# TencentARC/HOSNeRF

Measured on AMD Instinct MI355X. Metric: train rays/sec (stage3: forward + losses + backward + gradient all-reduce + Adam; LPIPS term OFF in this line -- stages.stage3_with_lpips carries it), higher is better.
Workload: dtype f32 (fp16/bf16 hi-lo split MFMA x3, fp32 accumulate)

## Files before the change

### hosnerf_amd/csrc/hos_mlpbwd.hip

```cpp
#include "hos_gemm_common.h"
#include <cstdlib>
#include <type_traits>
#include <utility>

namespace {

typedef __bf16 bf16x8 __attribute__((ext_vector_type(8)));
typedef __bf16 bf16x4 __attribute__((ext_vector_type(4)));
typedef short s16x4 __attribute__((ext_vector_type(4)));
typedef short s16x8 __attribute__((ext_vector_type(8)));

struct MlpBwdArgs {
    const float* dZ; int lddz;
    const float* X; int ldx;
    const float* W; int ldw;
    float* dX; int lddx;
    float* dW; int lddw;
    float* db;
    int M, N, K;
    int relu_mask;
    float* ws;
    int ws_dw;
    const int* m_dev;
};
// ... 272 lines not shown
                for (int q = 0; q < 4; ++q)
                    if (t * 4 + q < a.N) __hip_atomic_fetch_add(a.db + t * 4 + q, sv[q], __ATOMIC_RELAXED, __HIP_MEMORY_SCOPE_AGENT);
            }
        }
    }
#ifdef HOS_MB_TRACE
    asm volatile("s_waitcnt vmcnt(0)" ::: "memory");
    MB_STAMP();
#endif
#undef MB_STAMP
}

template <int KT>
__global__ __launch_bounds__(MB_NT, 1) void wgrad_tr_fast_kernel(MlpBwdArgs a) {
    constexpr int NT = 8, N_ = NT * 32, K_ = KT * 32, R = 32;
    constexpr int PZ = N_ * 2 + 32, PX = K_ * 2 + 32;
    constexpr int Z_PLANE = R * PZ, X_PLANE = R * PX;
    constexpr int ZU = R * (N_ / 4) / MB_NT;
    constexpr int XT = R * (K_ / 4);
    constexpr int XU = (XT + MB_NT - 1) / MB_NT;
    constexpr bool XALL = XT % MB_NT == 0;
    constexpr int WT = NT * KT, WPW = WT / 8;
    static_assert(WT % 8 == 0 && 8 % KT == 0, "a wave's WGRAD tiles share kt");

    extern __shared__ __attribute__((aligned(16))) char smem_mb[];
    char* const Zh = smem_mb;
    char* const Zl = Zh + Z_PLANE;
    char* const Xh = Zl + Z_PLANE;
    char* const Xl = Xh + X_PLANE;
    const int t = threadIdx.x, lane = t & 63, wave = t >> 6;
    const int tr_g = lane >> 4, tr_p = lane & 15;
    const int tr_row = 8 * (tr_g >> 1) + (tr_p >> 2);
    const int tr_col = 16 * (tr_g & 1) + 4 * (tr_p & 3);
    const bool xthread = XALL || t < XT;

    const int nrb = a.M / R;
    const int G = gridDim.x;
    float4 rzA[ZU], rxA[XU], rzB[ZU], rxB[XU];
    float4 bsum = make_float4(0.f, 0.f, 0.f, 0.f);
    auto gload = [&](float4 (&rz)[ZU], float4 (&rx)[XU], int rb) {
        rb = rb < nrb ? rb : nrb - 1;
        const float* zb = a.dZ + (size_t)rb * R * a.lddz;
        const float* xb = a.X + (size_t)rb * R * a.ldx;
#pragma unroll
        for (int i = 0; i < ZU; ++i) {
            const int u = t + MB_NT * i, row = u / (N_ / 4), c4 = u % (N_ / 4);
            rz[i] = ldg4(zb + (size_t)row * a.lddz + c4 * 4);
        }
#pragma unroll
        for (int i = 0; i < XU; ++i) {
            const int u = XALL ? t + MB_NT * i : (t < XT ? t : 0), row = u / (K_ / 4), c4 = u % (K_ / 4);
            rx[i] = ldg4(xb + (size_t)row * a.ldx + c4 * 4);
        }
    };
    auto sstore = [&](const float4 (&rz)[ZU], const float4 (&rx)[XU]) {
#pragma unroll
        for (int i = 0; i < ZU; ++i) {
            const int u = t + MB_NT * i, row = u / (N_ / 4), c4 = u % (N_ / 4);
            bsum.x += rz[i].x; bsum.y += rz[i].y; bsum.z += rz[i].z; bsum.w += rz[i].w;
            bf16x4 h, l;
            split4(rz[i], h, l);
            *reinterpret_cast<bf16x4*>(Zh + row * PZ + c4 * 8) = h;
            *reinterpret_cast<bf16x4*>(Zl + row * PZ + c4 * 8) = l;
        }
        if (xthread) {
#pragma unroll
            for (int i = 0; i < XU; ++i) {
                const int u = t + MB_NT * i, row = u / (K_ / 4), c4 = u % (K_ / 4);
                bf16x4 h, l;
                split4(rx[i], h, l);
                *reinterpret_cast<bf16x4*>(Xh + row * PX + c4 * 8) = h;
                *reinterpret_cast<bf16x4*>(Xl + row * PX + c4 * 8) = l;
            }
        }
    };
    f32x16 accW[WPW];
#pragma unroll
    for (int j = 0; j < WPW; ++j)
#pragma unroll
        for (int r = 0; r < 16; ++r) accW[j][r] = 0.f;
    auto compute = [&]() {
        const int kw = wave % KT;
        const char* xfrag = Xh + tr_row * PX + (kw * 32 + tr_col) * 2;
#pragma unroll
        for (int s = 0; s < R / 16; ++s) {
            const bf16x8 bh = tr_frag2(xfrag + s * 16 * PX, PX);
            const bf16x8 bl = tr_frag2(xfrag + X_PLANE + s * 16 * PX, PX);
#pragma unroll
            for (int j = 0; j < WPW; ++j) {
                const int ti = wave + 8 * j;
                const char* zfrag = Zh + tr_row * PZ + ((ti / KT) * 32 + tr_col) * 2;
                const bf16x8 ah = tr_frag2(zfrag + s * 16 * PZ, PZ);
                const bf16x8 al = tr_frag2(zfrag + Z_PLANE + s * 16 * PZ, PZ);
                accW[j] = mma3(ah, al, bh, bl, accW[j]);
            }
        }
    };
#define WG_BAR() asm volatile("s_waitcnt lgkmcnt(0)\n\ts_barrier" ::: "memory")
    auto step = [&](float4 (&rz)[ZU], float4 (&rx)[XU], const int rb) {
        sstore(rz, rx);
        WG_BAR();
        gload(rz, rx, rb + 2 * G);
        compute();
        WG_BAR();
    };
    int rb = blockIdx.x;
    gload(rzA, rxA, rb);
    gload(rzB, rxB, rb + G);
    step(rzA, rxA, rb);
    rb += G;
    if (rb < nrb) {
        step(rzB, rxB, rb);
        rb += G;
        while (rb + G < nrb) {
            step(rzA, rxA, rb);
            step(rzB, rxB, rb + G);
            rb += 2 * G;
        }
        if (rb < nrb) step(rzA, rxA, rb);
    }
#undef WG_BAR
    GemmArgs ew{};
    ew.C = a.ws + (size_t)blockIdx.x * (N_ * K_ + N_); ew.ldc = K_; ew.M = N_; ew.N = K_; ew.epi = HOS_EPI_NONE;
#pragma unroll
    for (int j = 0; j < WPW; ++j) {
        const int ti = wave + 8 * j;
        gemm_epilogue_tile<MODE_FWD>(ew, accW[j], (ti / KT) * 32, (ti % KT) * 32, lane);
    }
    if (a.db != nullptr) {
        float4* red = reinterpret_cast<float4*>(Zh);
        red[t] = bsum;
        __syncthreads();
        constexpr int CG = N_ / 4;
        if (t < CG) {
            float4 sacc = make_float4(0.f, 0.f, 0.f, 0.f);
            for (int k = t; k < MB_NT; k += CG) { const float4 v = red[k]; sacc.x += v.x; sacc.y += v.y; sacc.z += v.z; sacc.w += v.w; }
            *reinterpret_cast<float4*>(a.ws + (size_t)blockIdx.x * (N_ * K_ + N_) + N_ * K_ + t * 4) = sacc;
        }
    }
}

constexpr int MB_RSPLIT = 2;
__global__ __launch_bounds__(256) void mlp_bwd_reduce_kernel(const float* __restrict__ ws, int slabs, int n_, int k_, int nk, float* __restrict__ dW,
                                                             int lddw, float* __restrict__ db, int N, int K) {
    const int e = (blockIdx.x * 256 + threadIdx.x) * 4;
    const int slab = nk + n_;
    if (e >= slab || (e >= nk && db == nullptr)) return;
    float4 s = make_float4(0.f, 0.f, 0.f, 0.f);
    const int sy = gridDim.y;
    for (int g0 = blockIdx.y; g0 < slabs; g0 += 8 * sy) {
        float4 v[8];
#pragma unroll
        for (int i = 0; i < 8; ++i) {
            const int g = g0 + i * sy;
            v[i] = g < slabs ? *reinterpret_cast<const float4*>(ws + (size_t)g * slab + e) : make_float4(0.f, 0.f, 0.f, 0.f);
        }
#pragma unroll
        for (int i = 0; i < 8; ++i) { s.x += v[i].x; s.y += v[i].y; s.z += v[i].z; s.w += v[i].w; }
    }
    const float sv[4] = {s.x, s.y, s.z, s.w};
    if (e >= nk) {
#pragma unroll
        for (int q = 0; q < 4; ++q)
            if (e - nk + q < N) __hip_atomic_fetch_add(db + e - nk + q, sv[q], __ATOMIC_RELAXED, __HIP_MEMORY_SCOPE_AGENT);
        return;
    }
    const int n = e / k_, k = e % k_;
    if (n < N) {
#pragma unroll
        for (int q = 0; q < 4; ++q)
            if (k + q < K) __hip_atomic_fetch_add(dW + (size_t)n * lddw + k + q, sv[q], __ATOMIC_RELAXED, __HIP_MEMORY_SCOPE_AGENT);
    }
}

constexpr int MB_BATCH = 16;
struct ReduceJob { const float* ws; float* dW; float* db; int slabs, n_, k_, nk, lddw, N, K, first_block; };
struct ReduceBatch { ReduceJob j[MB_BATCH]; int count; };

__global__ __launch_bounds__(256) void mlp_bwd_reduce_batch_kernel(const ReduceBatch b) {
    int ji = 0;
#pragma unroll 1
    for (int i = 1; i < b.count; ++i) if ((int)blockIdx.x >= b.j[i].first_block) ji = i;
    const ReduceJob& J = b.j[ji];
    const int e = (((int)blockIdx.x - J.first_block) * 256 + threadIdx.x) * 4;
    const int slab = J.nk + J.n_;
    if (e >= slab || (e >= J.nk && J.db == nullptr)) return;
    float4 s = make_float4(0.f, 0.f, 0.f, 0.f);
    const int sy = gridDim.y;
    for (int g0 = blockIdx.y; g0 < J.slabs; g0 += 8 * sy) {
        float4 v[8];
#pragma unroll
        for (int i = 0; i < 8; ++i) {
            const int g = g0 + i * sy;
            v[i] = g < J.slabs ? *reinterpret_cast<const float4*>(J.ws + (size_t)g * slab + e) : make_float4(0.f, 0.f, 0.f, 0.f);
        }
#pragma unroll
        for (int i = 0; i < 8; ++i) { s.x += v[i].x; s.y += v[i].y; s.z += v[i].z; s.w += v[i].w; }
    }
    const float sv[4] = {s.x, s.y, s.z, s.w};
    if (e >= J.nk) {
#pragma unroll
        for (int q = 0; q < 4; ++q)
            if (e - J.nk + q < J.N) __hip_atomic_fetch_add(J.db + e - J.nk + q, sv[q], __ATOMIC_RELAXED, __HIP_MEMORY_SCOPE_AGENT);
        return;
    }
    const int n = e / J.k_, k = e % J.k_;
    if (n < J.N) {
#pragma unroll
        for (int q = 0; q < 4; ++q)
            if (k + q < J.K) __hip_atomic_fetch_add(J.dW + (size_t)n * J.lddw + k + q, sv[q], __ATOMIC_RELAXED, __HIP_MEMORY_SCOPE_AGENT);
    }
}

thread_local bool g_defer = false;
thread_local ReduceBatch g_batch = {};

static inline int reduce_split() {
    static const int v = getenv("HOS_MB_RSPLIT") ? atoi(getenv("HOS_MB_RSPLIT")) : MB_RSPLIT;
    return v > 0 ? v : MB_RSPLIT;
}

static int flush_reduce_batch(hipStream_t stream) {
    if (g_batch.count == 0) return 0;
    const ReduceJob& L = g_batch.j[g_batch.count - 1];
    const int blocks = L.first_block + hos_cdiv(L.nk + L.n_, 1024);
    hipLaunchKernelGGL(mlp_bwd_reduce_batch_kernel, dim3(blocks, reduce_split()), dim3(256), 0, stream, g_batch);
    g_batch.count = 0;
    return hos_launch_status();
}

template <int NT, int KT, bool DG>
int launch_mb(MlpBwdArgs a, size_t ws_floats, hipStream_t stream) {
    constexpr int N_ = NT * 32, K_ = KT * 32;
    constexpr int R = mb_rows(DG);
    constexpr size_t smem = (DG ? 2 * (size_t)N_ * (K_ * 2 + 32) : 0) + 2 * (size_t)R * (N_ * 2 + 32) + 2 * (size_t)R * (K_ * 2 + 32);
    static bool attr_set = false;
    if (!attr_set) {
        hipError_t e = hipFuncSetAttribute(reinterpret_cast<const void*>(&mlp_bwd_kernel<NT, KT, DG>),
                                           hipFuncAttributeMaxDynamicSharedMemorySize, (int)smem);
        if (e != hipSuccess) return (int)e;
        attr_set = true;
    }
    const int nrb = hos_cdiv(a.M, R);
    const int grid = nrb < 256 ? nrb : 256;
    a.ws_dw = 1;
    const int nk = a.ws_dw ? N_ * K_ : 0;
    if (a.ws != nullptr && (grid < 32 || ws_floats < (size_t)grid * (nk + N_) || (!a.ws_dw && a.db == nullptr))) a.ws = nullptr;
    hipLaunchKernelGGL((mlp_bwd_kernel<NT, KT, DG>), dim3(grid), dim3(MB_NT), smem, stream, a);
#ifndef HOS_MB_TRACE
    if (a.ws != nullptr) {
        if (g_defer) {
            if (g_batch.count == MB_BATCH) { const int rc = flush_reduce_batch(stream); if (rc != 0) return rc; }
            ReduceJob& J = g_batch.j[g_batch.count];
            J = ReduceJob{a.ws, a.dW, a.db, grid, N_, K_, nk, a.lddw, a.N, a.K,
                          g_batch.count ? g_batch.j[g_batch.count - 1].first_block + hos_cdiv(g_batch.j[g_batch.count - 1].nk + g_batch.j[g_batch.count - 1].n_, 1024) : 0};
            ++g_batch.count;
        } else {
            hipLaunchKernelGGL(mlp_bwd_reduce_kernel, dim3(hos_cdiv(nk + N_, 1024), reduce_split()), dim3(256), 0, stream,
                               a.ws, grid, N_, K_, nk, a.dW, a.lddw, a.db, a.N, a.K);
        }
    }
#endif
    return hos_launch_status();
}

template <int KT>
int launch_wgrad_fast(MlpBwdArgs a, size_t ws_floats, hipStream_t stream) {
    constexpr int N_ = 256, K_ = KT * 32, R = 32, nk = N_ * K_;
    constexpr size_t smem = 2 * (size_t)R * (N_ * 2 + 32) + 2 * (size_t)R * (K_ * 2 + 32);
    static const bool on = !(getenv("HOS_WGRAD_FAST") && atoi(getenv("HOS_WGRAD_FAST")) == 0);
    const int nrb = a.M / R;
    const int grid = nrb < 256 ? nrb : 256;
    if (!on || a.M % R != 0 || a.N != N_ || a.K != K_ || a.m_dev != nullptr || a.ws == nullptr || grid < 32 ||
        ws_floats < (size_t)grid * (nk + N_) || (((uintptr_t)a.ws) & 15u)) return -1;
    static bool attr_set = false;
    if (!attr_set) {
        hipError_t e = hipFuncSetAttribute(reinterpret_cast<const void*>(&wgrad_tr_fast_kernel<KT>), hipFuncAttributeMaxDynamicSharedMemorySize, (int)smem);
        if (e != hipSuccess) return (int)e;
        attr_set = true;
    }
    hipLaunchKernelGGL((wgrad_tr_fast_kernel<KT>), dim3(grid), dim3(MB_NT), smem, stream, a);
    if (g_defer) {
        if (g_batch.count == MB_BATCH) { const int rc = flush_reduce_batch(stream); if (rc != 0) return rc; }
        ReduceJob& J = g_batch.j[g_batch.count];
        J = ReduceJob{a.ws, a.dW, a.db, grid, N_, K_, nk, a.lddw, a.N, a.K,
                      g_batch.count ? g_batch.j[g_batch.count - 1].first_block + hos_cdiv(g_batch.j[g_batch.count - 1].nk + g_batch.j[g_batch.count - 1].n_, 1024) : 0};
        ++g_batch.count;
    } else {
        hipLaunchKernelGGL(mlp_bwd_reduce_kernel, dim3(hos_cdiv(nk + N_, 1024), reduce_split()), dim3(256), 0, stream,
                           a.ws, grid, N_, K_, nk, a.dW, a.lddw, a.db, a.N, a.K);
    }
    return hos_launch_status();
}

template <int NT, int KT, bool DG>
int64_t ws_floats_mb(int M) {
    const int nrb = hos_cdiv(M, mb_rows(DG));
    const int grid = nrb < 256 ? nrb : 256;
    return grid < 32 ? 0 : (int64_t)grid * (NT * 32 * KT * 32 + NT * 32);
}


typedef unsigned int u32x4 __attribute__((ext_vector_type(4)));
constexpr int CB_MAXS = 4;
constexpr int CB_R = 64;
constexpr int CB_W_BYTES = 2 * 128 * (128 * 2 + 32);
constexpr int CB_T_BYTES = 2 * CB_R * (128 * 2 + 32);
constexpr int CB_SMEM = CB_W_BYTES + 2 * CB_T_BYTES;

constexpr int cb_code(int nt, int kt, int mask, int out) { return nt | (kt << 4) | (mask << 8) | (out << 9); }
constexpr int cb_nt(int c) { return c & 15; }
constexpr int cb_kt(int c) { return (c >> 4) & 15; }
constexpr bool cb_mask(int c) { return (c >> 8) & 1; }
constexpr bool cb_out(int c) { return (c >> 9) & 1; }
constexpr int cb_image_bytes(int nt, int kt) { return ((2 * nt * 32 * (kt * 64 + 32)) + 8191) / 8192 * 8192; }

struct ChainBwdStep {
    const float* X; int ldx;
    const u32x4* Wp;
    float* dXout; int lddx;
    float* ws;
};
struct ChainBwdArgs {
    const float* dZ; int lddz;
    int M; const int* m_dev;
    ChainBwdStep st[CB_MAXS];
};

template <class F, int... I>
__device__ __forceinline__ void cb_static_for(F&& f, std::integer_sequence<int, I...>) { (f(std::integral_constant<int, I>{}), ...); }

template <int... CODE>
__global__ __launch_bounds__(MB_NT, 1) void chain_bwd_kernel(ChainBwdArgs a) {
    constexpr int S = sizeof...(CODE);
    constexpr int codes[S] = {CODE...};
    static_assert(S >= 1 && S <= CB_MAXS && cb_out(codes[S - 1]), "the last step of a group hands its dX over through HBM");
    constexpr int R = CB_R;
    constexpr auto wpw = [](int s) constexpr { return (cb_nt(codes[s]) * cb_kt(codes[s]) + 7) / 8; };
    constexpr auto acc_off = [wpw](int s) constexpr { int o = 0; for (int i = 0; i < s; ++i) o += wpw(i); return o; };
    constexpr int NACC = acc_off(S);
    constexpr auto zsrc = [](int s) constexpr { int v = -1; for (int i = 0; i < s; ++i) if (!cb_out(codes[i])) v = i; return v; };

    if (a.m_dev) a.M = min(a.M, *a.m_dev);
    extern __shared__ __attribute__((aligned(16))) char smem_mb[];
    char* const Wh = smem_mb;
    char* const Zh = smem_mb + CB_W_BYTES;
    char* const Xh = Zh + CB_T_BYTES;
    const int t = threadIdx.x, lane = t & 63, wave = t >> 6;
    const int l31 = lane & 31, lhi = lane >> 5;
    const int tr_g = lane >> 4, tr_p = lane & 15;
    const int tr_row = 8 * (tr_g >> 1) + (tr_p >> 2);
    const int tr_col = 16 * (tr_g & 1) + 4 * (tr_p & 3);

    constexpr int N0 = cb_nt(codes[0]) * 32;
    constexpr int ZU0 = R * (N0 / 4) / MB_NT;
    float4 rz[ZU0];
    float4 rx[4];
    u32x4 rw[9];
    float4 bsum = make_float4(0.f, 0.f, 0.f, 0.f);
    float4 zsum[S];
    f32x16 accW[NACC];
#pragma unroll
    for (int j = 0; j < NACC; ++j)
#pragma unroll
        for (int r = 0; r < 16; ++r) accW[j][r] = 0.f;
#pragma unroll
    for (int s = 0; s < S; ++s) zsum[s] = make_float4(0.f, 0.f, 0.f, 0.f);

    const int nrb = (a.M + R - 1) / R;
    const int G = gridDim.x;
    const int mlast = a.M - 1;

    auto uni = [](const void* p) {
        const uint64_t v = reinterpret_cast<uint64_t>(p);
        const uint32_t lo = __builtin_amdgcn_readfirstlane((uint32_t)v), hi = __builtin_amdgcn_readfirstlane((uint32_t)(v >> 32));
        return reinterpret_cast<const char*>(((uint64_t)hi << 32) | lo);
    };
    auto blk_rlast = [&](int rb) { return min(R - 1, mlast - rb * R); };
    auto gloadZ = [&](int rb) {
        rb = rb < nrb ? rb : nrb - 1;
        const char* base = uni(a.dZ + (size_t)rb * R * a.lddz);
        const int rlast = blk_rlast(rb);
#pragma unroll
        for (int i = 0; i < ZU0; ++i) {
            const int u = t + MB_NT * i, row = min(u / (N0 / 4), rlast), c4 = u % (N0 / 4);
            rz[i] = *reinterpret_cast<const float4*>(base + (unsigned)((row * a.lddz + c4 * 4) * 4));
        }
    };
    auto sstoreZ = [&](int rb) {
        constexpr int PZ = N0 * 2 + 32;
#pragma unroll
        for (int i = 0; i < ZU0; ++i) {
            const int u = t + MB_NT * i, row = u / (N0 / 4), c4 = u % (N0 / 4);
            float4 v = rz[i];
            if (rb * R + row >= a.M) v = make_float4(0.f, 0.f, 0.f, 0.f);
            bsum.x += v.x; bsum.y += v.y; bsum.z += v.z; bsum.w += v.w;
            bf16x4 h, l;
            split4(v, h, l);
            *reinterpret_cast<bf16x4*>(Zh + row * PZ + c4 * 8) = h;
            *reinterpret_cast<bf16x4*>(Zh + R * PZ + row * PZ + c4 * 8) = l;
        }
    };
    auto gloadX_part = [&](auto sc, int rb, int i0, int i1) {
        constexpr int s = decltype(sc)::value;
        constexpr int K_ = cb_kt(codes[s]) * 32, XU = R * (K_ / 4) / MB_NT;
        rb = rb < nrb ? rb : nrb - 1;
        const int ldx = a.st[s].ldx;
        const char* base = uni(a.st[s].X + (size_t)rb * R * ldx);
        const int rlast = blk_rlast(rb);
#pragma unroll
        for (int i = 0; i < XU; ++i) if (i >= i0 && i < i1) {
            const int u = t + MB_NT * i, row = min(u / (K_ / 4), rlast), c4 = u % (K_ / 4);
            rx[i] = *reinterpret_cast<const float4*>(base + (unsigned)((row * ldx + c4 * 4) * 4));
        }
    };
    auto gloadX = [&](auto sc, int rb) { gloadX_part(sc, rb, 0, 4); };
    auto sstoreX = [&](auto sc) {
        constexpr int s = decltype(sc)::value;
        constexpr int K_ = cb_kt(codes[s]) * 32, XU = R * (K_ / 4) / MB_NT, PX = K_ * 2 + 32;
#pragma unroll
        for (int i = 0; i < XU; ++i) {
            const int u = t + MB_NT * i, row = u / (K_ / 4), c4 = u % (K_ / 4);
            bf16x4 h, l;
            split4(rx[i], h, l);
            *reinterpret_cast<bf16x4*>(Xh + row * PX + c4 * 8) = h;
            *reinterpret_cast<bf16x4*>(Xh + R * PX + row * PX + c4 * 8) = l;
        }
    };
    const unsigned toff = (unsigned)t * 16u;
    auto loadW_part = [&](auto sc, int i0, int i1) {
        constexpr int s = decltype(sc)::value;
        constexpr int RW = cb_image_bytes(cb_nt(codes[s]), cb_kt(codes[s])) / 8192;
#pragma unroll
        for (int i = 0; i < RW; ++i) if (i >= i0 && i < i1) rw[i] = *reinterpret_cast<const u32x4*>(uni(reinterpret_cast<const char*>(a.st[s].Wp) + (size_t)i * 8192) + toff);
    };
    auto loadW = [&](auto sc) { loadW_part(sc, 0, 9); };
    auto storeW = [&](auto sc) {
        constexpr int s = decltype(sc)::value;
        constexpr int RW = cb_image_bytes(cb_nt(codes[s]), cb_kt(codes[s])) / 8192;
#pragma unroll
        for (int i = 0; i < RW; ++i) *reinterpret_cast<u32x4*>(Wh + i * 8192 + toff) = rw[i];
    };

    int rb = blockIdx.x;
    if (nrb > 0) {
        gloadZ(rb);
        gloadX(std::integral_constant<int, 0>{}, rb);
        loadW(std::integral_constant<int, 0>{});
    }

    for (; rb < nrb; rb += G) {
        sstoreZ(rb);
        sstoreX(std::integral_constant<int, 0>{});
        storeW(std::integral_constant<int, 0>{});
        __syncthreads();
        cb_static_for([&](auto sc) {
            constexpr int s = decltype(sc)::value;
            constexpr int code = codes[s];
            constexpr int NT = cb_nt(code), KT = cb_kt(code), N_ = NT * 32, K_ = KT * 32;
            constexpr int PZ = N_ * 2 + 32, PX = K_ * 2 + 32, PW = K_ * 2 + 32;
            constexpr int Z_PLANE = R * PZ, X_PLANE = R * PX, W_PLANE = N_ * PW;
            constexpr int DT = 2 * KT;
            constexpr int WT = NT * KT, WPW = (WT + 7) / 8;
            static_assert(s == 0 || !cb_out(codes[s > 0 ? s - 1 : 0]) ? true : true, "");
            constexpr int SN = s + 1 < S ? s + 1 : 0;
            constexpr int RWN = cb_image_bytes(cb_nt(codes[SN]), cb_kt(codes[SN])) / 8192;
            constexpr int XUN = R * (cb_kt(codes[SN]) * 32 / 4) / MB_NT;
            const int rbn = s + 1 < S ? rb : rb + G;
            f32x16 acc;
            const int rt = wave / KT, kt = wave % KT;
            const bool dg = wave < DT;
#pragma unroll
            for (int r = 0; r < 16; ++r) acc[r] = 0.f;
            {
                const char* zrow = Zh + (rt * 32 + l31) * PZ + lhi * 16;
                const char* wfrag = Wh + tr_row * PW + (kt * 32 + tr_col) * 2;
                constexpr int NK = N_ / 16;
#pragma unroll
                for (int k = 0; k < NK; ++k) {
                    if (dg) {
                        const bf16x8 ah = *reinterpret_cast<const bf16x8*>(zrow + k * 32);
                        const bf16x8 al = *reinterpret_cast<const bf16x8*>(zrow + Z_PLANE + k * 32);
                        const bf16x8 bh = tr_frag2(wfrag + k * 16 * PW, PW);
                        const bf16x8 bl = tr_frag2(wfrag + W_PLANE + k * 16 * PW, PW);
#ifndef HOS_CB_EXP_NOMFMA
                        acc = mma3(ah, al, bh, bl, acc);
#else
                        acc[k & 15] += (float)ah[0] + (float)al[1] + (float)bh[2] + (float)bl[3];
#endif
                    }
#ifndef HOS_CB_EXP_NOW
                    loadW_part(std::integral_constant<int, SN>{}, k * RWN / NK, (k + 1) * RWN / NK);
#endif
                    __builtin_amdgcn_sched_barrier(0);
                }
            }
            {
                const int kw = wave % KT;
                const char* xfrag = Xh + tr_row * PX + (kw * 32 + tr_col) * 2;
                constexpr int NK = R / 16;
#pragma unroll
                for (int k = 0; k < NK; ++k) {
                    if (wave < WT) {
                        const bf16x8 bh = tr_frag2(xfrag + k * 16 * PX, PX);
                        const bf16x8 bl = tr_frag2(xfrag + X_PLANE + k * 16 * PX, PX);
#pragma unroll
                        for (int j = 0; j < WPW; ++j) {
                            const int ti = wave + 8 * j;
                            if (ti < WT) {
                                const char* zfrag = Zh + tr_row * PZ + ((ti / KT) * 32 + tr_col) * 2;
                                const bf16x8 ah = tr_frag2(zfrag + k * 16 * PZ, PZ);
                                const bf16x8 al = tr_frag2(zfrag + Z_PLANE + k * 16 * PZ, PZ);
#ifndef HOS_CB_EXP_NOMFMA
                                accW[acc_off(s) + j] = mma3(ah, al, bh, bl, accW[acc_off(s) + j]);
#else
                                accW[acc_off(s) + j][k & 15] += (float)ah[0] + (float)al[1] + (float)bh[2] + (float)bl[3];
#endif
                            }
                        }
                    }
                    gloadX_part(std::integral_constant<int, SN>{}, rbn, k * XUN / NK, (k + 1) * XUN / NK);
                    __builtin_amdgcn_sched_barrier(0);
                }
            }
            if constexpr (s + 1 == S) gloadZ(rb + G);
            float v[4][4];
            if (dg) {
                const int q = l31 & 3;
                const int colb = kt * 32 + (l31 & ~3);
#pragma unroll
                for (int g = 0; g < 4; ++g) {
                    float v0 = acc[4 * g + 0], v1 = acc[4 * g + 1], v2 = acc[4 * g + 2], v3 = acc[4 * g + 3];
                    {
                        const float s0 = (q & 1) ? v0 : v1, s1 = (q & 1) ? v2 : v3;
                        const float r0 = quad_xor1(s0), r1 = quad_xor1(s1);
                        if (q & 1) { v0 = r0; v2 = r1; } else { v1 = r0; v3 = r1; }
                        const float t0 = (q & 2) ? v0 : v2, t1 = (q & 2) ? v1 : v3;
                        const float u0 = quad_xor2(t0), u1 = quad_xor2(t1);
                        if (q & 2) { v0 = u0; v1 = u1; } else { v2 = u0; v3 = u1; }
                    }
                    v[g][0] = v0; v[g][1] = v1; v[g][2] = v2; v[g][3] = v3;
                    const int lrow = rt * 32 + q + 8 * g + 4 * lhi;
                    if constexpr (cb_mask(code)) {
                        const uint2 m = *reinterpret_cast<const uint2*>(Xh + lrow * PX + colb * 2);
                        const uint32_t h[4] = {m.x & 0xffffu, m.x >> 16, m.y & 0xffffu, m.y >> 16};
#pragma unroll
                        for (int c = 0; c < 4; ++c)
                            if ((h[c] & 0x8000u) || (h[c] & 0x7fffu) == 0) v[g][c] = 0.f;
                    }
                    if constexpr (cb_out(code)) {
                        const int lddx = a.st[s].lddx;
                        char* ob = const_cast<char*>(uni(a.st[s].dXout + (size_t)rb * R * lddx));
                        if (rb * R + lrow < a.M)
                            *reinterpret_cast<float4*>(ob + (unsigned)((lrow * lddx + colb) * 4)) = make_float4(v[g][0], v[g][1], v[g][2], v[g][3]);
                    } else {
                        zsum[s].x += v[g][0]; zsum[s].y += v[g][1]; zsum[s].z += v[g][2]; zsum[s].w += v[g][3];
                    }
                }
            }
            if constexpr (s + 1 < S) {
                __syncthreads();
                if constexpr (!cb_out(code)) {
                    constexpr int PZn = K_ * 2 + 32;
                    static_assert(cb_nt(codes[s + 1 < S ? s + 1 : s]) == KT || cb_out(code), "step shapes do not chain");
                    if (wave < DT) {
                        const int q = l31 & 3;
                        const int colb = kt * 32 + (l31 & ~3);
#pragma unroll
                        for (int g = 0; g < 4; ++g) {
                            const int lrow = rt * 32 + q + 8 * g + 4 * lhi;
                            bf16x4 h, l;
                            split4(make_float4(v[g][0], v[g][1], v[g][2], v[g][3]), h, l);
                            *reinterpret_cast<bf16x4*>(Zh + lrow * PZn + colb * 2) = h;
                            *reinterpret_cast<bf16x4*>(Zh + R * PZn + lrow * PZn + colb * 2) = l;
                        }
                    }
                }
                sstoreX(std::integral_constant<int, s + 1 < S ? s + 1 : 0>{});
#ifndef HOS_CB_EXP_NOW
                storeW(std::integral_constant<int, s + 1 < S ? s + 1 : 0>{});
#endif
                __syncthreads();
            }
        }, std::make_integer_sequence<int, S>{});
        __syncthreads();
    }

    cb_static_for([&](auto sc) {
        constexpr int s = decltype(sc)::value;
        constexpr int NT = cb_nt(codes[s]), KT = cb_kt(codes[s]), N_ = NT * 32, K_ = KT * 32;
        constexpr int WT = NT * KT, WPW = (WT + 7) / 8;
        GemmArgs ew{};
        ew.C = a.st[s].ws + (size_t)blockIdx.x * (N_ * K_ + N_); ew.ldc = K_; ew.M = N_; ew.N = K_; ew.epi = HOS_EPI_NONE;
#pragma unroll
        for (int j = 0; j < WPW; ++j) {
            const int ti = wave + 8 * j;
            if (ti < WT) gemm_epilogue_tile<MODE_FWD>(ew, accW[acc_off(s) + j], (ti / KT) * 32, (ti % KT) * 32, lane);
        }
    }, std::make_integer_sequence<int, S>{});
    float4* red = reinterpret_cast<float4*>(Zh);
    {
        red[t] = bsum;
        __syncthreads();
        constexpr int CG = N0 / 4;
        float4 sacc = make_float4(0.f, 0.f, 0.f, 0.f);
        if (t < CG)
            for (int k = t; k < MB_NT; k += CG) { const float4 x = red[k]; sacc.x += x.x; sacc.y += x.y; sacc.z += x.z; sacc.w += x.w; }
        cb_static_for([&](auto sc) {
            constexpr int s = decltype(sc)::value;
            constexpr int N_ = cb_nt(codes[s]) * 32, K_ = cb_kt(codes[s]) * 32;
            if constexpr (zsrc(s) == -1)
                if (t < CG) *reinterpret_cast<float4*>(a.st[s].ws + (size_t)blockIdx.x * (N_ * K_ + N_) + N_ * K_ + t * 4) = sacc;
        }, std::make_integer_sequence<int, S>{});
        __syncthreads();
    }
    cb_static_for([&](auto pc) {
        constexpr int p = decltype(pc)::value;
        if constexpr (!cb_out(codes[p])) {
            constexpr int KTp = cb_kt(codes[p]), CG = KTp * 8;
            red[t] = (wave < 2 * KTp) ? zsum[p] : make_float4(0.f, 0.f, 0.f, 0.f);
            __syncthreads();
            float4 sacc = make_float4(0.f, 0.f, 0.f, 0.f);
            if (t < CG) {
                const int kt = t >> 3, cq = t & 7;
#pragma unroll
                for (int rt = 0; rt < 2; ++rt)
#pragma unroll
                    for (int hh = 0; hh < 2; ++hh)
#pragma unroll
                        for (int q = 0; q < 4; ++q) {
                            const float4 x = red[(rt * KTp + kt) * 64 + hh * 32 + cq * 4 + q];
                            sacc.x += x.x; sacc.y += x.y; sacc.z += x.z; sacc.w += x.w;
                        }
            }
            cb_static_for([&](auto sc) {
                constexpr int s = decltype(sc)::value;
                constexpr int N_ = cb_nt(codes[s]) * 32, K_ = cb_kt(codes[s]) * 32;
                if constexpr (zsrc(s) == p)
                    if (t < CG) *reinterpret_cast<float4*>(a.st[s].ws + (size_t)blockIdx.x * (N_ * K_ + N_) + N_ * K_ + t * 4) = sacc;
            }, std::make_integer_sequence<int, S>{});
            __syncthreads();
        }
    }, std::make_integer_sequence<int, S>{});
}

struct ChainBwdPackJob { const float* W; int ldw, N, K, nt, kt; uint16_t* image; };
struct ChainBwdPackJobs { ChainBwdPackJob j[8]; };
__global__ __launch_bounds__(256) void chain_bwd_pack_kernel(const ChainBwdPackJobs jobs) {
    const ChainBwdPackJob& J = jobs.j[blockIdx.y];
    const int N_ = J.nt * 32, K_ = J.kt * 32, pw = K_ + 16;
    const int total = cb_image_bytes(J.nt, J.kt) / 2;
    for (int e = blockIdx.x * 256 + threadIdx.x; e < total; e += gridDim.x * 256) {
        const int plane = e / (N_ * pw), r = e % (N_ * pw);
        const int n = r / pw, k = r % pw;
        uint16_t out = 0;
        if (plane < 2 && n < J.N && k < J.K) {
            const float w = J.W[(size_t)n * J.ldw + k];
            const __bf16 hi = (__bf16)w;
            out = plane == 0 ? __builtin_bit_cast(uint16_t, hi) : __builtin_bit_cast(uint16_t, (__bf16)(w - (float)hi));
        }
        J.image[e] = out;
    }
}

struct ChainBwdCfg { int S; int code[CB_MAXS]; };
constexpr int CB_NCFG = 4;
constexpr ChainBwdCfg CB_CFG[CB_NCFG] = {
    {2, {cb_code(1, 4, 1, 0), cb_code(4, 4, 1, 1), 0, 0}},
    {3, {cb_code(4, 2, 0, 1), cb_code(4, 4, 1, 0), cb_code(4, 4, 1, 1), 0}},
    {3, {cb_code(4, 4, 1, 0), cb_code(4, 4, 1, 0), cb_code(4, 2, 0, 1), 0}},
    {3, {cb_code(4, 4, 1, 0), cb_code(4, 4, 1, 0), cb_code(4, 4, 0, 1), 0}},
};

template <int... CODE>
int launch_chain_bwd(const ChainBwdArgs& a, int grid, hipStream_t stream) {
    static bool attr_set = false;
    if (!attr_set) {
        hipError_t e = hipFuncSetAttribute(reinterpret_cast<const void*>(&chain_bwd_kernel<CODE...>), hipFuncAttributeMaxDynamicSharedMemorySize, CB_SMEM);
        if (e != hipSuccess) return (int)e;
        attr_set = true;
    }
    hipLaunchKernelGGL((chain_bwd_kernel<CODE...>), dim3(grid), dim3(MB_NT), CB_SMEM, stream, a);
    return hos_launch_status();
}

}

extern "C" int hos_linear_bwd_fused(const float* dZ, int lddz, const float* X, int ldx, const float* W, int ldw,
                                    float* dX, int lddx, float* dW, int lddw, float* db, int M, int N, int K,
                                    int relu_mask, float* ws, int64_t ws_floats, const int32_t* rows_dev, hos_stream_t stream) {
    if (!dZ || !X || !W || !dW || M <= 0 || N <= 0 || K <= 0 || ws_floats < 0) return HOS_E_ARG;
    if (N > 128 || K > 128) return HOS_E_SHAPE;
    if ((lddz & 3) || (ldx & 3) || (ldw & 3) || (K & 3) || (dX && (lddx & 3))) return HOS_E_ALIGN;
    if (((uintptr_t)dZ | (uintptr_t)X | (uintptr_t)W | (uintptr_t)ws) & 15u) return HOS_E_ALIGN;
    MlpBwdArgs a{dZ, lddz, X, ldx, W, ldw, dX, lddx, dW, lddw, db, M, N, K, relu_mask, ws, 1, rows_dev};
    hipStream_t s = static_cast<hipStream_t>(stream);
    const int nt = hos_cdiv(N, 32), kt = hos_cdiv(K, 32);
    if (nt <= 1 && kt <= 4) return launch_mb<1, 4, true>(a, (size_t)ws_floats, s);
    if (kt <= 2) return launch_mb<4, 2, true>(a, (size_t)ws_floats, s);
    return launch_mb<4, 4, true>(a, (size_t)ws_floats, s);
}

extern "C" int hos_linear_wgrad_tr(const float* dZ, int lddz, const float* X, int ldx, float* dW, int lddw, float* db,
                                   int M, int N, int K, float* ws, int64_t ws_floats, hos_stream_t stream) {
    if (!dZ || !X || !dW || M <= 0 || N <= 0 || K <= 0) return HOS_E_ARG;
    if (N > 256 || K > 256) return HOS_E_SHAPE;
    if ((lddz & 3) || (ldx & 3) || (K & 3)) return HOS_E_ALIGN;
    if (((uintptr_t)dZ | (uintptr_t)X) & 15u) return HOS_E_ALIGN;
    MlpBwdArgs a{dZ, lddz, X, ldx, nullptr, 0, nullptr, 0, dW, lddw, db, M, N, K, 0, ws, 0};
    hipStream_t s = static_cast<hipStream_t>(stream);
    const int kt = hos_cdiv(K, 32);
    if (N == 256 && (K == 256 || K == 64)) {
        const int rc = K == 256 ? launch_wgrad_fast<8>(a, (size_t)ws_floats, s) : launch_wgrad_fast<2>(a, (size_t)ws_floats, s);
        if (rc >= 0) return rc;
    }
    if (kt <= 4) return launch_mb<8, 4, false>(a, (size_t)ws_floats, s);
    return launch_mb<8, 8, false>(a, (size_t)ws_floats, s);
}

extern "C" int hos_mlp_bwd_defer(int on) { g_defer = on != 0; return 0; }

extern "C" int hos_mlp_bwd_flush(hos_stream_t stream) { return flush_reduce_batch(static_cast<hipStream_t>(stream)); }

extern "C" long long hos_mlp_bwd_ws_floats(int M, int N, int K, int fused) {
    if (M <= 0 || N <= 0 || K <= 0) return 0;
    const int nt = hos_cdiv(N, 32), kt = hos_cdiv(K, 32);
    if (fused) {
        if (nt <= 1 && kt <= 4) return ws_floats_mb<1, 4, true>(M);
        if (kt <= 2) return ws_floats_mb<4, 2, true>(M);
        return ws_floats_mb<4, 4, true>(M);
    }
    return kt <= 4 ? ws_floats_mb<8, 4, false>(M) : ws_floats_mb<8, 8, false>(M);
}

extern "C" int hos_mlp_chain_bwd_steps(int cfg) { return cfg >= 0 && cfg < CB_NCFG ? CB_CFG[cfg].S : HOS_E_ARG; }

extern "C" long long hos_mlp_chain_bwd_image_bytes(int cfg, int step) {
    if (cfg < 0 || cfg >= CB_NCFG || step < 0 || step >= CB_CFG[cfg].S) return 0;
    return cb_image_bytes(cb_nt(CB_CFG[cfg].code[step]), cb_kt(CB_CFG[cfg].code[step]));
}

extern "C" long long hos_mlp_chain_bwd_ws_floats(int cfg, int M) {
    if (cfg < 0 || cfg >= CB_NCFG || M <= 0) return 0;
    const int nrb = hos_cdiv(M, CB_R), grid = nrb < 256 ? nrb : 256;
    long long f = 0;
    for (int s = 0; s < CB_CFG[cfg].S; ++s) {
        const int n_ = cb_nt(CB_CFG[cfg].code[s]) * 32, k_ = cb_kt(CB_CFG[cfg].code[s]) * 32;
        f += (long long)grid * (n_ * k_ + n_);
    }
    return f;
}

extern "C" int hos_mlp_chain_bwd_pack(int n, const int* cfg, const int* step, const float* const* W, const int* ldw, const int* N,
                                      const int* K, void* const* image, hos_stream_t stream) {
    if (n <= 0 || n > 8 || !cfg || !step || !W || !ldw || !N || !K || !image) return HOS_E_ARG;
    ChainBwdPackJobs jobs{};
    for (int i = 0; i < n; ++i) {
        if (cfg[i] < 0 || cfg[i] >= CB_NCFG || step[i] < 0 || step[i] >= CB_CFG[cfg[i]].S || !W[i] || !image[i] || N[i] <= 0 || K[i] <= 0) return HOS_E_ARG;
        const int nt = cb_nt(CB_CFG[cfg[i]].code[step[i]]), kt = cb_kt(CB_CFG[cfg[i]].code[step[i]]);
        if (N[i] > nt * 32 || K[i] > kt * 32 || ldw[i] < K[i]) return HOS_E_SHAPE;
        if ((uintptr_t)image[i] & 15u) return HOS_E_ALIGN;
        jobs.j[i] = ChainBwdPackJob{W[i], ldw[i], N[i], K[i], nt, kt, static_cast<uint16_t*>(image[i])};
    }
    hipLaunchKernelGGL(chain_bwd_pack_kernel, dim3(36, n), dim3(256), 0, static_cast<hipStream_t>(stream), jobs);
    return hos_launch_status();
}

extern "C" int hos_mlp_chain_bwd(int cfg, const float* dZ, int lddz, int M, const int32_t* rows_dev, const float* const* X, const int* ldx,
                                 const void* const* images, float* const* dXout, const int* lddx, float* const* dW, const int* lddw,
                                 float* const* db, const int* N, const int* K, float* ws, int64_t ws_floats, hos_stream_t stream) {
    if (cfg < 0 || cfg >= CB_NCFG || !dZ || M <= 0 || !X || !ldx || !images || !dXout || !lddx || !dW || !lddw || !db || !N || !K || !ws) return HOS_E_ARG;
    const ChainBwdCfg& C = CB_CFG[cfg];
    if (ws_floats < hos_mlp_chain_bwd_ws_floats(cfg, M)) return HOS_E_SHAPE;
    if (((uintptr_t)dZ | (uintptr_t)ws) & 15u) return HOS_E_ALIGN;
    if (lddz < cb_nt(C.code[0]) * 32 || (lddz & 3)) return HOS_E_SHAPE;
    const int nrb = hos_cdiv(M, CB_R), grid = nrb < 256 ? nrb : 256;
    ChainBwdArgs a{};
    a.dZ = dZ; a.lddz = lddz; a.M = M; a.m_dev = rows_dev;
    float* wsp = ws;
    ReduceJob jobs[CB_MAXS];
    for (int s = 0; s < C.S; ++s) {
        const int n_ = cb_nt(C.code[s]) * 32, k_ = cb_kt(C.code[s]) * 32;
        if (!X[s] || !images[s] || !dW[s] || N[s] <= 0 || K[s] <= 0 || N[s] > n_ || K[s] > k_) return HOS_E_ARG;
        if (ldx[s] < k_ || (ldx[s] & 3) || (((uintptr_t)X[s] | (uintptr_t)images[s]) & 15u)) return HOS_E_ALIGN;
        if (cb_out(C.code[s])) {
            if (!dXout[s] || lddx[s] < k_ || (lddx[s] & 3) || ((uintptr_t)dXout[s] & 15u)) return HOS_E_ALIGN;
        }
        a.st[s].X = X[s]; a.st[s].ldx = ldx[s]; a.st[s].Wp = static_cast<const u32x4*>(images[s]);
        a.st[s].dXout = dXout[s]; a.st[s].lddx = lddx[s]; a.st[s].ws = wsp;
        jobs[s] = ReduceJob{wsp, dW[s], db[s], grid, n_, k_, n_ * k_, lddw[s], N[s], K[s], 0};
        wsp += (size_t)grid * (n_ * k_ + n_);
    }
    hipStream_t st = static_cast<hipStream_t>(stream);
    int rc;
    switch (cfg) {
        case 0: rc = launch_chain_bwd<CB_CFG[0].code[0], CB_CFG[0].code[1]>(a, grid, st); break;
        case 1: rc = launch_chain_bwd<CB_CFG[1].code[0], CB_CFG[1].code[1], CB_CFG[1].code[2]>(a, grid, st); break;
        case 2: rc = launch_chain_bwd<CB_CFG[2].code[0], CB_CFG[2].code[1], CB_CFG[2].code[2]>(a, grid, st); break;
        default: rc = launch_chain_bwd<CB_CFG[3].code[0], CB_CFG[3].code[1], CB_CFG[3].code[2]>(a, grid, st); break;
    }
    if (rc != 0) return rc;
    for (int s = 0; s < C.S; ++s) {
        if (g_defer) {
            if (g_batch.count == MB_BATCH) { const int r2 = flush_reduce_batch(st); if (r2 != 0) return r2; }
            ReduceJob& J = g_batch.j[g_batch.count];
            J = jobs[s];
            J.first_block = g_batch.count ? g_batch.j[g_batch.count - 1].first_block + hos_cdiv(g_batch.j[g_batch.count - 1].nk + g_batch.j[g_batch.count - 1].n_, 1024) : 0;
            ++g_batch.count;
        } else {
            const ReduceJob& J = jobs[s];
            hipLaunchKernelGGL(mlp_bwd_reduce_kernel, dim3(hos_cdiv(J.nk + J.n_, 1024), reduce_split()), dim3(256), 0, st,
                               J.ws, J.slabs, J.n_, J.k_, J.nk, J.dW, J.lddw, J.db, J.N, J.K);
        }
    }
    return hos_launch_status();
}
```

Baseline: 134,300.

## Stream chain-backward weight images into LDS via global_load_lds DMA

Adds a DMA variant of the chained MLP backward kernel, on by default and switchable off with an environment variable. Weight images are copied straight into LDS with global_load_lds instead of staging through nine VGPR registers. The dW MMA loop is rewritten with inline ds_read_b64_tr_b16 and counted lgkmcnt waits. The epilogue is moved ahead of the MMA loop, and barriers use explicit waitcnt plus s_barrier. The goal is to free registers and overlap weight and X prefetch with the MFMA work, at the cost of hand-placed waits that could be mis-synchronised.

```diff
diff --git a/hosnerf_amd/csrc/hos_mlpbwd.hip b/hosnerf_amd/csrc/hos_mlpbwd.hip
--- a/hosnerf_amd/csrc/hos_mlpbwd.hip
+++ b/hosnerf_amd/csrc/hos_mlpbwd.hip
@@ -598,6 +598,7 @@
 
 
 typedef unsigned int u32x4 __attribute__((ext_vector_type(4)));
+typedef float cb_f4 __attribute__((ext_vector_type(4)));
 constexpr int CB_MAXS = 4;
 constexpr int CB_R = 64;
 constexpr int CB_W_BYTES = 2 * 128 * (128 * 2 + 32);
@@ -626,7 +627,19 @@
 template <class F, int... I>
 __device__ __forceinline__ void cb_static_for(F&& f, std::integer_sequence<int, I...>) { (f(std::integral_constant<int, I>{}), ...); }
 
-template <int... CODE>
+__device__ __forceinline__ void cb_dma16(const void* gsrc, void* ldst) {
+    __builtin_amdgcn_global_load_lds((const __attribute__((address_space(1))) void*)gsrc,
+                                     (__attribute__((address_space(3))) void*)ldst, 16, 0, 0);
+}
+#define CB_RDTR(DST, ADDR, OFF) asm volatile("ds_read_b64_tr_b16 %0, %1 offset:%2" : "=v"(DST) : "v"(ADDR), "n"(OFF))
+#define CB_BAR() asm volatile("s_waitcnt lgkmcnt(0)\n\ts_barrier" ::: "memory")
+constexpr int CB_VMCNT0 = 0x0F70;
+__device__ __forceinline__ bf16x8 cb_join(const s16x4& a, const s16x4& b) {
+    const s16x8 j = __builtin_shufflevector(a, b, 0, 1, 2, 3, 4, 5, 6, 7);
+    return __builtin_bit_cast(bf16x8, j);
+}
+
+template <bool DMA, int... CODE>
 __global__ __launch_bounds__(MB_NT, 1) void chain_bwd_kernel(ChainBwdArgs a) {
     constexpr int S = sizeof...(CODE);
     constexpr int codes[S] = {CODE...};
@@ -652,7 +665,7 @@
     constexpr int ZU0 = R * (N0 / 4) / MB_NT;
     float4 rz[ZU0];
     float4 rx[4];
-    u32x4 rw[9];
+    u32x4 rw[DMA ? 1 : 9];
     float4 bsum = make_float4(0.f, 0.f, 0.f, 0.f);
     float4 zsum[S];
     f32x16 accW[NACC];
@@ -671,6 +684,16 @@
         const uint64_t v = reinterpret_cast<uint64_t>(p);
         const uint32_t lo = __builtin_amdgcn_readfirstlane((uint32_t)v), hi = __builtin_amdgcn_readfirstlane((uint32_t)(v >> 32));
         return reinterpret_cast<const char*>(((uint64_t)hi << 32) | lo);
+    };
+    auto ld16 = [](const char* p) {
+        if constexpr (DMA) {
+            const cb_f4 x = *reinterpret_cast<const __attribute__((address_space(1))) cb_f4*>((uint64_t)p);
+            return make_float4(x[0], x[1], x[2], x[3]);
+        } else return *reinterpret_cast<const float4*>(p);
+    };
+    auto st16 = [](char* p, const float4& x) {
+        if constexpr (DMA) *reinterpret_cast<__attribute__((address_space(1))) cb_f4*>((uint64_t)p) = cb_f4{x.x, x.y, x.z, x.w};
+        else *reinterpret_cast<float4*>(p) = x;
     };
     auto blk_rlast = [&](int rb) { return min(R - 1, mlast - rb * R); };
     auto gloadZ = [&](int rb) {
@@ -680,7 +703,7 @@
 #pragma unroll
         for (int i = 0; i < ZU0; ++i) {
             const int u = t + MB_NT * i, row = min(u / (N0 / 4), rlast), c4 = u % (N0 / 4);
-            rz[i] = *reinterpret_cast<const float4*>(base + (unsigned)((row * a.lddz + c4 * 4) * 4));
+            rz[i] = ld16(base + (unsigned)((row * a.lddz + c4 * 4) * 4));
         }
     };
     auto sstoreZ = [&](int rb) {
@@ -707,7 +730,7 @@
 #pragma unroll
         for (int i = 0; i < XU; ++i) if (i >= i0 && i < i1) {
             const int u = t + MB_NT * i, row = min(u / (K_ / 4), rlast), c4 = u % (K_ / 4);
-            rx[i] = *reinterpret_cast<const float4*>(base + (unsigned)((row * ldx + c4 * 4) * 4));
+            rx[i] = ld16(base + (unsigned)((row * ldx + c4 * 4) * 4));
         }
     };
     auto gloadX = [&](auto sc, int rb) { gloadX_part(sc, rb, 0, 4); };
@@ -727,25 +750,40 @@
     auto loadW_part = [&](auto sc, int i0, int i1) {
         constexpr int s = decltype(sc)::value;
         constexpr int RW = cb_image_bytes(cb_nt(codes[s]), cb_kt(codes[s])) / 8192;
-#pragma unroll
-        for (int i = 0; i < RW; ++i) if (i >= i0 && i < i1) rw[i] = *reinterpret_cast<const u32x4*>(uni(reinterpret_cast<const char*>(a.st[s].Wp) + (size_t)i * 8192) + toff);
+        if constexpr (!DMA) {
+#pragma unroll
+            for (int i = 0; i < RW; ++i) if (i >= i0 && i < i1) rw[i] = *reinterpret_cast<const u32x4*>(uni(reinterpret_cast<const char*>(a.st[s].Wp) + (size_t)i * 8192) + toff);
+        }
     };
     auto loadW = [&](auto sc) { loadW_part(sc, 0, 9); };
     auto storeW = [&](auto sc) {
         constexpr int s = decltype(sc)::value;
         constexpr int RW = cb_image_bytes(cb_nt(codes[s]), cb_kt(codes[s])) / 8192;
-#pragma unroll
-        for (int i = 0; i < RW; ++i) *reinterpret_cast<u32x4*>(Wh + i * 8192 + toff) = rw[i];
-    };
+        if constexpr (!DMA) {
+#pragma unroll
+            for (int i = 0; i < RW; ++i) *reinterpret_cast<u32x4*>(Wh + i * 8192 + toff) = rw[i];
+        }
+    };
+    const int wave_u = __builtin_amdgcn_readfirstlane(wave);
+    auto dmaW_part = [&](auto sc, int i0, int i1) {
+        constexpr int s = decltype(sc)::value;
+        constexpr int RW = cb_image_bytes(cb_nt(codes[s]), cb_kt(codes[s])) / 8192;
+#pragma unroll
+        for (int i = 0; i < RW; ++i) if (i >= i0 && i < i1)
+            cb_dma16(uni(reinterpret_cast<const char*>(a.st[s].Wp) + (size_t)i * 8192) + toff, Wh + i * 8192 + wave_u * 1024);
+    };
+    const unsigned lds_base = (unsigned)(uintptr_t)(__attribute__((address_space(3))) char*)smem_mb;
 
     int rb = blockIdx.x;
     if (nrb > 0) {
         gloadZ(rb);
         gloadX(std::integral_constant<int, 0>{}, rb);
-        loadW(std::integral_constant<int, 0>{});
+        if constexpr (DMA) dmaW_part(std::integral_constant<int, 0>{}, 0, 9);
+        else loadW(std::integral_constant<int, 0>{});
     }
 
     for (; rb < nrb; rb += G) {
+        if constexpr (DMA) __builtin_amdgcn_s_waitcnt(CB_VMCNT0);
         sstoreZ(rb);
         sstoreX(std::integral_constant<int, 0>{});
         storeW(std::integral_constant<int, 0>{});
@@ -791,6 +829,86 @@
                     __builtin_amdgcn_sched_barrier(0);
                 }
             }
+            float v[4][4];
+            auto epilogue = [&]() {
+                if (dg) {
+                    const int q = l31 & 3;
+                    const int colb = kt * 32 + (l31 & ~3);
+#pragma unroll
+                    for (int g = 0; g < 4; ++g) {
+                        float v0 = acc[4 * g + 0], v1 = acc[4 * g + 1], v2 = acc[4 * g + 2], v3 = acc[4 * g + 3];
+                        {
+                            const float s0 = (q & 1) ? v0 : v1, s1 = (q & 1) ? v2 : v3;
+                            const float r0 = quad_xor1(s0), r1 = quad_xor1(s1);
+                            if (q & 1) { v0 = r0; v2 = r1; } else { v1 = r0; v3 = r1; }
+                            const float t0 = (q & 2) ? v0 : v2, t1 = (q & 2) ? v1 : v3;
+                            const float u0 = quad_xor2(t0), u1 = quad_xor2(t1);
+                            if (q & 2) { v0 = u0; v1 = u1; } else { v2 = u0; v3 = u1; }
+                        }
+                        v[g][0] = v0; v[g][1] = v1; v[g][2] = v2; v[g][3] = v3;
+                        const int lrow = rt * 32 + q + 8 * g + 4 * lhi;
+                        if constexpr (cb_mask(code)) {
+                            const uint2 m = *reinterpret_cast<const uint2*>(Xh + lrow * PX + colb * 2);
+                            const uint32_t h[4] = {m.x & 0xffffu, m.x >> 16, m.y & 0xffffu, m.y >> 16};
+#pragma unroll
+                            for (int c = 0; c < 4; ++c)
+                                if ((h[c] & 0x8000u) || (h[c] & 0x7fffu) == 0) v[g][c] = 0.f;
+                        }
+                        if constexpr (cb_out(code)) {
+                            const int lddx = a.st[s].lddx;
+                            char* ob = const_cast<char*>(uni(a.st[s].dXout + (size_t)rb * R * lddx));
+                            if (rb * R + lrow < a.M)
+                                st16(ob + (unsigned)((lrow * lddx + colb) * 4), make_float4(v[g][0], v[g][1], v[g][2], v[g][3]));
+                        } else {
+                            zsum[s].x += v[g][0]; zsum[s].y += v[g][1]; zsum[s].z += v[g][2]; zsum[s].w += v[g][3];
+                        }
+                    }
+                }
+            };
+            if constexpr (DMA) {
+                epilogue();
+                CB_BAR();
+                const int kw = wave % KT;
+                const unsigned ax = lds_base + (unsigned)(CB_W_BYTES + CB_T_BYTES) + (unsigned)(tr_row * PX + (kw * 32 + tr_col) * 2);
+                const unsigned az = lds_base + (unsigned)CB_W_BYTES + (unsigned)(tr_row * PZ + ((wave / KT) * 32 + tr_col) * 2);
+                constexpr int ZJ = (8 / KT) * 64;
+                constexpr int NK = R / 16;
+#pragma unroll
+                for (int k = 0; k < NK; ++k) {
+                    if (WT >= 8 || wave < WT) {
+                        s16x4 xf[4], zf[WPW][4];
+                        CB_RDTR(xf[0], ax, k * 16 * PX);
+                        CB_RDTR(xf[1], ax, k * 16 * PX + 4 * PX);
+                        CB_RDTR(xf[2], ax, X_PLANE + k * 16 * PX);
+                        CB_RDTR(xf[3], ax, X_PLANE + k * 16 * PX + 4 * PX);
+#pragma unroll
+                        for (int j = 0; j < WPW; ++j) {
+                            CB_RDTR(zf[j][0], az, j * ZJ + k * 16 * PZ);
+                            CB_RDTR(zf[j][1], az, j * ZJ + k * 16 * PZ + 4 * PZ);
+                            CB_RDTR(zf[j][2], az, j * ZJ + Z_PLANE + k * 16 * PZ);
+                            CB_RDTR(zf[j][3], az, j * ZJ + Z_PLANE + k * 16 * PZ + 4 * PZ);
+                        }
+                        static_assert(WPW == 1 || WPW == 2, "counted waits below");
+                        if constexpr (WPW == 2)
+                            asm volatile("s_waitcnt lgkmcnt(4)" : "+v"(xf[0]), "+v"(xf[1]), "+v"(xf[2]), "+v"(xf[3]),
+                                         "+v"(zf[0][0]), "+v"(zf[0][1]), "+v"(zf[0][2]), "+v"(zf[0][3]));
+                        else
+                            asm volatile("s_waitcnt lgkmcnt(0)" : "+v"(xf[0]), "+v"(xf[1]), "+v"(xf[2]), "+v"(xf[3]),
+                                         "+v"(zf[0][0]), "+v"(zf[0][1]), "+v"(zf[0][2]), "+v"(zf[0][3]));
+                        const bf16x8 bh = cb_join(xf[0], xf[1]), bl = cb_join(xf[2], xf[3]);
+                        accW[acc_off(s)] = mma3(cb_join(zf[0][0], zf[0][1]), cb_join(zf[0][2], zf[0][3]), bh, bl, accW[acc_off(s)]);
+                        if constexpr (WPW == 2) {
+                            asm volatile("s_waitcnt lgkmcnt(0)" : "+v"(zf[WPW - 1][0]), "+v"(zf[WPW - 1][1]), "+v"(zf[WPW - 1][2]), "+v"(zf[WPW - 1][3]));
+                            accW[acc_off(s) + WPW - 1] = mma3(cb_join(zf[WPW - 1][0], zf[WPW - 1][1]), cb_join(zf[WPW - 1][2], zf[WPW - 1][3]), bh, bl,
+                                                              accW[acc_off(s) + WPW - 1]);
+                        }
+                    }
+                    __builtin_amdgcn_sched_barrier(0);
+                    dmaW_part(std::integral_constant<int, SN>{}, k * RWN / NK, (k + 1) * RWN / NK);
+                    gloadX_part(std::integral_constant<int, SN>{}, rbn, k * XUN / NK, (k + 1) * XUN / NK);
+                    __builtin_amdgcn_sched_barrier(0);
+                }
+            } else
             {
                 const int kw = wave % KT;
                 const char* xfrag = Xh + tr_row * PX + (kw * 32 + tr_col) * 2;
@@ -820,41 +938,12 @@
                 }
             }
             if constexpr (s + 1 == S) gloadZ(rb + G);
-            float v[4][4];
-            if (dg) {
-                const int q = l31 & 3;
-                const int colb = kt * 32 + (l31 & ~3);
-#pragma unroll
-                for (int g = 0; g < 4; ++g) {
-                    float v0 = acc[4 * g + 0], v1 = acc[4 * g + 1], v2 = acc[4 * g + 2], v3 = acc[4 * g + 3];
-                    {
-                        const float s0 = (q & 1) ? v0 : v1, s1 = (q & 1) ? v2 : v3;
-                        const float r0 = quad_xor1(s0), r1 = quad_xor1(s1);
-                        if (q & 1) { v0 = r0; v2 = r1; } else { v1 = r0; v3 = r1; }
-                        const float t0 = (q & 2) ? v0 : v2, t1 = (q & 2) ? v1 : v3;
-                        const float u0 = quad_xor2(t0), u1 = quad_xor2(t1);
-                        if (q & 2) { v0 = u0; v1 = u1; } else { v2 = u0; v3 = u1; }
-                    }
-                    v[g][0] = v0; v[g][1] = v1; v[g][2] = v2; v[g][3] = v3;
-                    const int lrow = rt * 32 + q + 8 * g + 4 * lhi;
-                    if constexpr (cb_mask(code)) {
-                        const uint2 m = *reinterpret_cast<const uint2*>(Xh + lrow * PX + colb * 2);
-                        const uint32_t h[4] = {m.x & 0xffffu, m.x >> 16, m.y & 0xffffu, m.y >> 16};
-#pragma unroll
-                        for (int c = 0; c < 4; ++c)
-                            if ((h[c] & 0x8000u) || (h[c] & 0x7fffu) == 0) v[g][c] = 0.f;
-                    }
-                    if constexpr (cb_out(code)) {
-                        const int lddx = a.st[s].lddx;
-                        char* ob = const_cast<char*>(uni(a.st[s].dXout + (size_t)rb * R * lddx));
-                        if (rb * R + lrow < a.M)
-                            *reinterpret_cast<float4*>(ob + (unsigned)((lrow * lddx + colb) * 4)) = make_float4(v[g][0], v[g][1], v[g][2], v[g][3]);
-                    } else {
-                        zsum[s].x += v[g][0]; zsum[s].y += v[g][1]; zsum[s].z += v[g][2]; zsum[s].w += v[g][3];
-                    }
-                }
-            }
+            if constexpr (!DMA) epilogue();
             if constexpr (s + 1 < S) {
+                if constexpr (DMA) {
+                    CB_BAR();
+                    __builtin_amdgcn_s_waitcnt(CB_VMCNT0);
+                } else
                 __syncthreads();
                 if constexpr (!cb_out(code)) {
                     constexpr int PZn = K_ * 2 + 32;
@@ -882,6 +971,7 @@
         __syncthreads();
     }
 
+    if constexpr (DMA) __builtin_amdgcn_s_waitcnt(CB_VMCNT0);
     cb_static_for([&](auto sc) {
         constexpr int s = decltype(sc)::value;
         constexpr int NT = cb_nt(codes[s]), KT = cb_kt(codes[s]), N_ = NT * 32, K_ = KT * 32;
@@ -968,15 +1058,15 @@
     {3, {cb_code(4, 4, 1, 0), cb_code(4, 4, 1, 0), cb_code(4, 4, 0, 1), 0}},
 };
 
-template <int... CODE>
+template <bool DMA, int... CODE>
 int launch_chain_bwd(const ChainBwdArgs& a, int grid, hipStream_t stream) {
     static bool attr_set = false;
     if (!attr_set) {
-        hipError_t e = hipFuncSetAttribute(reinterpret_cast<const void*>(&chain_bwd_kernel<CODE...>), hipFuncAttributeMaxDynamicSharedMemorySize, CB_SMEM);
+        hipError_t e = hipFuncSetAttribute(reinterpret_cast<const void*>(&chain_bwd_kernel<DMA, CODE...>), hipFuncAttributeMaxDynamicSharedMemorySize, CB_SMEM);
         if (e != hipSuccess) return (int)e;
         attr_set = true;
     }
-    hipLaunchKernelGGL((chain_bwd_kernel<CODE...>), dim3(grid), dim3(MB_NT), CB_SMEM, stream, a);
+    hipLaunchKernelGGL((chain_bwd_kernel<DMA, CODE...>), dim3(grid), dim3(MB_NT), CB_SMEM, stream, a);
     return hos_launch_status();
 }
 
@@ -1088,13 +1178,18 @@
         wsp += (size_t)grid * (n_ * k_ + n_);
     }
     hipStream_t st = static_cast<hipStream_t>(stream);
+    const char* const dma_env = getenv("HOS_CHAIN_BWD_DMA");
+    const bool dma = !(dma_env && atoi(dma_env) == 0);
     int rc;
-    switch (cfg) {
-        case 0: rc = launch_chain_bwd<CB_CFG[0].code[0], CB_CFG[0].code[1]>(a, grid, st); break;
-        case 1: rc = launch_chain_bwd<CB_CFG[1].code[0], CB_CFG[1].code[1], CB_CFG[1].code[2]>(a, grid, st); break;
-        case 2: rc = launch_chain_bwd<CB_CFG[2].code[0], CB_CFG[2].code[1], CB_CFG[2].code[2]>(a, grid, st); break;
-        default: rc = launch_chain_bwd<CB_CFG[3].code[0], CB_CFG[3].code[1], CB_CFG[3].code[2]>(a, grid, st); break;
-    }
+#define CB_LAUNCH(D) \
+    switch (cfg) { \
+        case 0: rc = launch_chain_bwd<D, CB_CFG[0].code[0], CB_CFG[0].code[1]>(a, grid, st); break; \
+        case 1: rc = launch_chain_bwd<D, CB_CFG[1].code[0], CB_CFG[1].code[1], CB_CFG[1].code[2]>(a, grid, st); break; \
+        case 2: rc = launch_chain_bwd<D, CB_CFG[2].code[0], CB_CFG[2].code[1], CB_CFG[2].code[2]>(a, grid, st); break; \
+        default: rc = launch_chain_bwd<D, CB_CFG[3].code[0], CB_CFG[3].code[1], CB_CFG[3].code[2]>(a, grid, st); break; \
+    }
+    if (dma) { CB_LAUNCH(true) } else { CB_LAUNCH(false) }
+#undef CB_LAUNCH
     if (rc != 0) return rc;
     for (int s = 0; s < C.S; ++s) {
         if (g_defer) {
```

After: 133,900. About the same (-0.3%).
